# treangenlab/bronko

Measured on AMD Instinct MI355X. Metric: reads/sec through call k-mer->pileup, SARS-CoV-2 k=21, higher is better.
Workload: dtype u64

## Files before the change

### bronko_amd/csrc/bk_engine.cpp

```cpp
#include <hip/hip_runtime.h>

#include <algorithm>
#include <cstdarg>
#include <cstdio>
#include <cstdlib>
#include <cstring>
#include <memory>
#include <string>
#include <vector>

#include "../host/lcb.hpp"
#include "bk_engine.h"

thread_local std::string g_err;

int fail(int code, const char* fmt, ...) {
    char buf[1024];
    va_list ap;
    va_start(ap, fmt);
    vsnprintf(buf, sizeof buf, fmt, ap);
    va_end(ap);
    g_err = buf;
    return code;
}
// ... 32 lines not shown
    BK_HIP(e->n_deferred.alloc(2));
    if (prm->pileup_selected_only && ix.ent_files.p) BK_HIP(e->deferred_mask.alloc(e->deferred.n));
    if (!e->sparse) {
        BK_HIP(e->deferred_n.alloc(e->deferred.n));
        for (MatePlane& p : e->mate) BK_HIP(hipMemset(p.counters.p, 0, std::max<size_t>(p.counters.n, 1) * sizeof(unsigned long long)));
    }
    if (ix.n_files == 1 && !e->sparse && ix.n_full > 0) { BK_HIP(e->lean_e_list.alloc((size_t)ix.n_full)); BK_HIP(e->lean_n_list.alloc(8)); BK_HIP(hipMemset(e->lean_n_list.p, 0, 8 * sizeof(unsigned int))); }
    BK_HIP(e->pileup.alloc(ix.total_cells * 4 * 4));
    e->gather_mode = ix.gather_ok && e->sparse && ix.cell_file.p && ix.dirty_ans.p && ix.W > 1 && ix.file_cell_lo_d.p && !test_env("BK_NO_GATHER");
    if (e->gather_mode) {
        for (MatePlane& p : e->mate) BK_HIP(p.alias_hits.alloc((size_t)bk_engine::kAliasCap * 3));
        BK_HIP(e->n_alias_hits.alloc(2));
        BK_HIP(e->last_sel.upload(std::vector<int>(1, -1)));
        BK_HIP(hipMemset(e->pileup.p, 0, std::max<size_t>(e->pileup.n, 1) * sizeof(unsigned long long)));
        const bool two_pass = prm->pileup_selected_only != 0 && ix.n_files > 1;
        if (!two_pass && prm->cs < (1ull << 28) && ix.total_cells >= 2 * (uint64_t)ix.n_full && !test_env("BK_NO_VOTE_TABLE")) {
            BK_HIP(e->row_bits.alloc((size_t)((bk::v_real_rows(ix.n_full, ix.v_span) + 31) / 32) + 1));
            BK_HIP(e->vote_tab.alloc(bk::vote_table_words(ix.view())));
        }
    }
    BK_HIP(e->stats.alloc((size_t)2 * ix.n_files * 3));
    BK_HIP(e->present.alloc((size_t)2 * ix.n_files));
    if (prm->pileup_selected_only != 0 && ix.n_files > 1) BK_HIP(e->sel_out.alloc(1));
    BK_HIP(e->l2_plan.alloc(4));
    BK_HIP(e->kstats.alloc(8));
    e->use_items = !e->sparse && ix.ref_in_lds && ix.W > 0 && ix.n_lds_bins > 0 && !test_env("BK_NO_ITEMS") && ix.seed_tab2.p && ix.rc_words.p &&
                   bk::item_geometry(std::min<uint32_t>(ix.n_lds_bins, (uint32_t)ix.total_cells), ix.n_full, ix.v_span, &e->ig) &&
                   bk::items_lds_bytes(e->ig, std::min<uint32_t>(ix.n_lds_bins, (uint32_t)ix.total_cells)) <= 128u * 1024u;
    if (e->use_items) {
        if (const char* cp = test_env("BK_ITEM_CAPS")) {
            unsigned ce = 0, cv = 0;
            if (sscanf(cp, "%u,%u", &ce, &cv) == 2 && ce >= 8 && cv >= 8 && ce <= 64 && cv <= 64 && ce % 8 == 0 && cv % 8 == 0) {
                bk::ItemGeom g2 = e->ig;
                g2.cap_e = ce; g2.cap_v = cv; g2.wg_items = g2.n_ebins * ce + g2.n_vbins * cv; g2.wg_stride = g2.wg_items;
                if (bk::items_lds_bytes(g2, std::min<uint32_t>(ix.n_lds_bins, (uint32_t)ix.total_cells)) <= 118u * 1024u) e->ig = g2;
            }
        }
        const size_t g = bk::items_max_grid(ix.n_cus);
        e->ig.grid_max = (uint32_t)g;
        BK_HIP(e->items.alloc(g * e->ig.wg_stride + 64));
        BK_HIP(e->item_tab.alloc(g * ((size_t)e->ig.n_ebins + e->ig.n_vbins)));
        BK_HIP(e->item_gext.alloc(g * ((size_t)e->ig.n_ebins + e->ig.n_vbins) * bk::kItemGCap));
        BK_HIP(e->ov.alloc((size_t)1 << 20));
        BK_HIP(e->ov_n.alloc(4));
        BK_HIP(hipMemset(e->ov_n.p, 0, 4 * sizeof(unsigned long long)));
    } else {
        BK_HIP(e->slabs.alloc((size_t)ix.n_cus * std::max<uint32_t>(ix.n_lds_bins, 1)));
// ... 280 lines not shown
                        m2[0] / n2, m2[1] / n2, m2[2] / n2, m2[3] / n2);
        if (test_env("BK_L2_STATS")[0] == '2')
            for (int b = 0; b < n_wg; b++) fprintf(stderr, "[bk]   wg %d: %.1f %.1f %.1f %.1f\n", b, (clk[4 * b] - t0) * 0.01, (clk[4 * b + 1] - t0) * 0.01, (clk[4 * b + 2] - t0) * 0.01, (clk[4 * b + 3] - t0) * 0.01);
    }
    fprintf(stderr, "[bk] finalize: %u + %u k-mers deferred to the general kernel\n", nd[0], nd[1]);
    if (e->gather_mode) {
        unsigned int ah[2] = {0u, 0u};
        BK_HIP(hipMemcpy(ah, e->n_alias_hits.p, sizeof ah, hipMemcpyDeviceToHost));
        fprintf(stderr, "[bk] votes gathered cell by cell (bk_gather.hip); alias hits among the deferred k-mers: %u + %u\n", ah[0], ah[1]);
    }
    if (e->sparse) {
        unsigned int nl[8];
        BK_HIP(hipMemcpy(nl, e->mate[0].n_list.p, sizeof nl, hipMemcpyDeviceToHost));
        fprintf(stderr, "[bk] sparse finalize (mate file 0): %u V rows of %llu, %u pseudo rows of %llu, %u reference k-mers of %u and %u pseudo k-mers of %u touched\n",
                nl[0], (unsigned long long)bk::v_real_rows(ix.n_full, ix.v_span), nl[4], (unsigned long long)ix.n_prows, nl[2], ix.n_full, nl[3], ix.n_u - ix.n_full);
    }
    fprintf(stderr, "[bk] scan: %llu mismatches counted, %llu items processed, %llu E gaps before a mismatch, %llu behind the last\n", h[23], h[24], h[25], h[26]);
    fprintf(stderr, "[bk] scan N batches: %llu with %llu pieces (%.1f per batch), %llu of them forced by a tile's end\n", h[20], h[21], h[20] ? (double)h[21] / (double)h[20] : 0.0, h[22]);
    fprintf(stderr, "[bk] scan marked: no-diagonal %llu, dirty-head %llu, clean-head %llu, pairs %llu | level 2: k-mers %llu in %llu chunks, simple %llu, dead %llu, "
            "dirty answers %llu (one difference but id unknown: %llu), neither half present %llu, slow %llu (diffs 0/1/2/3+ with a diagonal: %llu/%llu/%llu/%llu) -> member %llu, neighbour %llu, nothing %llu\n",
            h[0], h[1], h[2], h[3], h[4], h[11], h[5], h[6], h[16], h[17], h[18], h[7], h[12], h[13], h[14], h[15], h[8], h[9], h[10]);
    return BK_OK;
}
#else
static int l2_count_report(bk_engine*, const bk::ScanArgs&) { return BK_OK; }
static int l2_stats_arm(bk_engine*) { return BK_OK; }
static int l2_stats_report(bk_engine*) { return BK_OK; }
#endif

static bk::ScanArgs scan_args(const bk_engine* e, int mate, const uint32_t* d_words, uint32_t stride_words, const uint16_t* d_lens, uint64_t n,
                              const unsigned long long* n_records_dev) {
    const IndexTables& ix = *e->ix;
    const MatePlane& pl = e->mate[mate];
    bk::ScanArgs a{};
    a.n_records_dev = n_records_dev; a.ixp = ix.d_view.p;
    a.k = ix.k; a.wstart = ix.wstart; a.W = ix.W; a.v_omin = ix.v_omin; a.v_span = ix.v_span; a.v_off = ix.v_off; a.total_cells = (uint32_t)ix.total_cells; a.n_u = ix.n_u;
    a.ref_words = ix.ref_words.p; a.cell_codes = ix.cell_codes.p; a.cell_has = ix.cell_has.p; a.cell_clean = ix.cell_clean.p; a.cell_clean3 = ix.cell_clean3.p; a.cell_yf = ix.cell_yf.p; a.cell_yr = ix.cell_yr.p; a.id_at = ix.id_at.p; a.cell_fast = ix.cell_fast.p; a.cell_nat = ix.cell_nat.p; a.cell_natrow = ix.cell_natrow.p; a.cell_blk = ix.cell_blk.p; a.seed_tab = ix.seed_tab.p; a.seed_log2 = ix.seed_log2;
    a.seed_tab2 = ix.seed_tab2.p; a.seed2_log2 = ix.seed2_log2; a.rc_words = ix.rc_words.p;
    a.n_direct = e->use_items && ix.n_files == 1 && ix.max_seqs_per_file == 1 && (uint64_t)ix.n_lds_bins >= ix.total_cells && !test_env("BK_NO_N_DIRECT");
    a.words = d_words; a.lens = d_lens; a.n_records = n; a.stride_words = stride_words;
    a.counters = pl.counters.p; a.kmer_total = e->kstats.p + mate * 4 + 1;
    a.ablate = ix.ablate; a.slabs = e->slabs.p; a.n_lds_bins = ix.n_lds_bins; a.ref_in_lds = ix.ref_in_lds ? 1 : 0;
    a.ktab_keys = e->ktab.keys.p; a.ktab_cnt = e->ktab.cnt.p; a.ktab_log2 = e->ktab.log2;
    a.ktab_overflow = e->ktab_out.p + 4; a.mate = (uint32_t)mate;
    a.occ = ix.occ.p; a.n_files = ix.n_files;
    if (e->sparse) {
        a.touch_v = pl.touch_v.p; a.touch_b = pl.touch_b.p; a.touch_p = pl.touch_p.p; a.touch_e = pl.touch_e.p;
        a.rl_recip = ~0ull / (unsigned long long)(ix.v_span + 1) + 1ull;
    }
    a.dbg = e->dbg.p; a.l2_words = bk::scan_l2_words(stride_words, ix.k); a.l2_min_grid = (uint32_t)std::max(1, ix.n_cus / 2);
    if (e->use_items) { a.ig = e->ig; a.items = e->items.p; a.tab = e->item_tab.p; a.gext = e->item_gext.p; a.ov = e->ov.p; a.ov_n = e->ov_n.p; a.ov_cap = (uint32_t)e->ov.n; }
    return a;
}
static int choose_window(bk_engine* e, bk::ScanArgs& a, uint64_t n) {
    const IndexTables& ix = *e->ix;
    if (ix.occ.p && !e->win_chosen && n > 0) {
        BK_HIP(hipMemsetAsync(e->win_votes.p, 0, e->win_votes.n * sizeof(unsigned int), e->stream));
        const char* wf = test_env("BK_WINDOW_FILE");
        const int forced = wf ? std::max(0, atoi(wf)) : -1;
        bk::launch_pick_window(a, 16384, e->win_votes.p, ix.file_cell_lo_d.p, forced, e->win_sel.p, e->stream);
        e->win_chosen = true;
    }
    a.win_dev = ix.occ.p ? e->win_sel.p : nullptr;
    return BK_OK;
}
static uint64_t next_launch(const bk_engine* e, uint64_t left, uint64_t l2_cap, uint32_t& grid) {
    const IndexTables& ix = *e->ix;
    grid = bk::scan_grid(left, ix.n_cus);
    uint64_t take = e->use_items ? std::min<uint64_t>(left, l2_cap) : std::min<uint64_t>(std::min<uint64_t>(left, bk::scan_max_records(grid)), l2_cap);
    if (ix.max_launch_records) take = std::min<uint64_t>(take, ix.max_launch_records);
    if (e->use_items) {
        int share = ix.n_cus - ix.n_cus / 4;
        if (const char* fr = test_env("BK_ITEM_SHARE")) share = std::max(1, std::min(ix.n_cus, ix.n_cus * atoi(fr) / 16));
        grid = bk::items_grid(take, ix.family.load() > 1 ? share : ix.n_cus);
        if (const char* gr = test_env("BK_ITEM_GRID")) grid = std::max<uint32_t>(1, std::min<uint32_t>(grid, (uint32_t)atoi(gr)));
    }
    return take;
}
static int make_l2_room(bk_engine* e, bk::ScanArgs& a, uint64_t l2_cap) {
    if (e->l2_bits.n < a.n_records * a.l2_words || e->l2_diag.n < a.n_records) {
        BK_HIP(hipStreamSynchronize(e->stream));
        const uint64_t recs = std::min<uint64_t>(std::max<uint64_t>(a.n_records + a.n_records / 4, 1 << 16), l2_cap);
        BK_HIP(e->l2_bits.alloc((size_t)recs * a.l2_words)); BK_HIP(e->n_bits.alloc((size_t)recs * a.l2_words)); BK_HIP(e->l2_diag.alloc((size_t)recs));
        BK_HIP(e->l2_any.alloc((size_t)(recs + 31) / 32)); BK_HIP(e->n_any.alloc((size_t)(recs + 31) / 32));
        for (DevBuf<unsigned int>* b : {&e->l2_bits, &e->l2_any, &e->n_bits, &e->n_any}) BK_HIP(hipMemsetAsync(b->p, 0, b->n * sizeof(unsigned int), e->stream));
    }
    a.l2_bits = e->l2_bits.p; a.l2_diag = e->l2_diag.p; a.l2_any = e->l2_any.p; a.n_bits = e->n_bits.p; a.n_any = e->n_any.p;
    return BK_OK;
}
static int bin_items(bk_engine* e, bk::ScanArgs& a, int mate, uint32_t grid, bool wait_v) {
    const IndexTables& ix = *e->ix;
    MatePlane& pl = e->mate[mate];
    bk_engine::Span sp(e, 3);
    bk::BinArgs b{};
    b.ig = e->ig; b.items = e->items.p; b.tab = e->item_tab.p; b.gext = e->item_gext.p; b.n_wg = grid; b.ov = e->ov.p; b.ov_n = e->ov_n.p; b.ov_cap = (uint32_t)e->ov.n;
    b.ov_par = e->ov_par; e->ov_par ^= 1u;
    b.id_at = ix.id_at.p; b.cell_codes = ix.cell_codes.p + bk::scan_ref_pad_words(); b.win_lo = a.win_lo; b.win_dev = a.win_dev; b.total_cells = (uint32_t)ix.total_cells;
    b.counters = pl.counters.p; b.v_off = ix.v_off; b.v_real_len = bk::v_real_len(ix.n_full, ix.v_span); b.rl = (uint32_t)ix.v_span + 1u;
    const bool v_clean = pl.take_v_clean();
    b.v_mode = ix.item_v_mode >= 0 ? ix.item_v_mode : (v_clean ? 2 : 1);
    if (const char* ba = test_env("BK_BIN_ABLATE")) b.ablate = atoi(ba);
    if (wait_v) {
        e->pending.on = true; e->pending.mate = mate; e->pending.b = b;
        b.part = 1;
        a.touch_v = pl.fuse_touch.p; a.rl_recip = ~0ull / (unsigned long long)(ix.v_span + 1) + 1ull;
        pl.items_wait();
    } else {
        pl.no_more_waiting();
        if (e->fuse_ok) a.touch_v = nullptr;
    }
    BK_HIP(bk::launch_bin_count(b, e->stream));
    return BK_OK;
}
static int level2_and_fold(bk_engine* e, const bk::ScanArgs& a, int mate, uint32_t grid) {
    const IndexTables& ix = *e->ix;
    bk_engine::Span sp(e, 3);
    if (int rc = l2_count_report(e, a)) return rc;
    if (ix.ablate == 1 || ix.ablate == 4) {
        BK_HIP(hipMemsetAsync(e->n_bits.p, 0, (size_t)a.n_records * a.l2_words * sizeof(unsigned int), e->stream));
        BK_HIP(hipMemsetAsync(e->n_any.p, 0, e->n_any.n * sizeof(unsigned int), e->stream));
    }
    else BK_HIP(bk::launch_level2(a, ix.n_cus, e->stream));
    if (!e->use_items) {
        bk::FoldArgs f{};
        f.slabs = e->slabs.p; f.n_slabs = grid; f.n_lds_bins = ix.n_lds_bins; f.id_at = ix.id_at.p; f.cell_codes = ix.cell_codes.p + bk::scan_ref_pad_words(); f.win_lo = a.win_lo; f.win_dev = a.win_dev; f.touch_e = a.touch_e;
        f.counters = e->mate[mate].counters.p;
        bk::launch_fold(f, e->stream);
    }
    return BK_OK;
}
static int push_device(bk_engine* e, int mate, const uint32_t* d_words, uint32_t stride_words, const uint16_t* d_lens, uint64_t n,
                       const unsigned long long* n_records_dev = nullptr, uint64_t kmers_upper = 0) {
    MatePlane& pl = e->mate[mate];
    if (int rc = pl.zero_if_stale(e)) return rc;
    const uint64_t upper = kmers_upper ? kmers_upper : n * (uint64_t)stride_words * 16;
    if (int rc = ensure_ktab_room(e, upper)) return rc;
    if (e->dump) { if (int rc = dump_push(e, mate, d_words, stride_words, d_lens, n, n_records_dev, upper)) return rc; }
    pl.written();
    if (int rc = l2_stats_arm(e)) return rc;
    bk::ScanArgs a = scan_args(e, mate, d_words, stride_words, d_lens, n, n_records_dev);
    if (e->ix->W <= 0) {
        bk::launch_count_kmers(a, e->stream);
    } else {
        if (int rc = choose_window(e, a, n)) return rc;
        const uint64_t l2_cap = std::max<uint64_t>(64, ((1ull << 30) / sizeof(unsigned int)) / a.l2_words);
        for (uint64_t base = 0; base < n; base += a.n_records) {
            uint32_t grid = 0;
            a.rec_base = base; a.n_records = next_launch(e, n - base, l2_cap, grid);
            if (int rc = make_l2_room(e, a, l2_cap)) return rc;
            if (int rc = flush_pending_items(e)) return rc;
            const bool wait_v = e->fuse_ok && a.n_direct && !pl.fuse_off && e->ix->item_v_mode < 0;
            a.l2_plan = e->use_items && e->ix->n_files == 1 && e->ix->family.load() >= 4 && !test_env("BK_NO_L2_PLAN") ? e->l2_plan.p : nullptr;
            {
                bk_engine::Span sp(e, 0);
                if (e->use_items) { a.ov_par = e->ov_par; BK_HIP(bk::launch_scan_items(a, grid, e->stream)); }
                else BK_HIP(bk::launch_scan_count(a, grid, e->stream));
            }
            if (e->use_items) { if (int rc = bin_items(e, a, mate, grid, wait_v)) return rc; }
            if (int rc = level2_and_fold(e, a, mate, grid)) return rc;
        }
    }
    BK_HIP(hipGetLastError());
    if (!n_records_dev) pl.pushed_records += n;
    return note_ktab_fill(e);
}

static constexpr int kPush = 1;
static int push_checks(bk_engine* e, int mate, uint64_t n, bool batch_ok, const char* bad_batch, bool too_large) {
    if (!e) return fail(BK_ERR_INVALID, "null engine");
    if (!e->in_sample) return fail(BK_ERR_STATE, "bk_push_reads_* called before bk_sample_begin");
    if (mate < 0 || mate > 1) return fail(BK_ERR_INVALID, "mate must be 0 or 1");
    if (n == 0) return BK_OK;
    if (!batch_ok) return fail(BK_ERR_INVALID, "%s", bad_batch);
    if (too_large) return fail(BK_ERR_INVALID, "batch too large: push at most 2^32 bases per call");
    BK_HIP(hipSetDevice(e->device));
    return kPush;
}
static int packed_checks(bk_engine* e, int mate, const void* words, uint32_t stride_words, const void* lens, uint64_t n) {
    return push_checks(e, mate, n, words && lens && stride_words != 0 && stride_words <= 4096, "bad record batch",
                       stride_words != 0 && n > (1ull << 32) / ((uint64_t)stride_words * 16));
}
struct PackGeom {
// ... 781 lines not shown
```

### bronko_amd/csrc/bk_engine.h

```cpp
#pragma once
#include <hip/hip_runtime.h>

#include <algorithm>
#include <atomic>
#include <chrono>
#include <cstdio>
#include <cstdlib>
#include <memory>
#include <string>
#include <thread>
#include <vector>

#include "../../include/bronko_hip.h"
#include "bk_device.h"
#include "bk_kernels.h"

#pragma GCC visibility push(hidden)

extern thread_local std::string g_err;

int fail(int code, const char* fmt, ...);

#define BK_HIP(expr)                                                                                  \
    do {                                                                                              \
// ... 210 lines not shown
    DevBuf<unsigned int> xchg_cnt;
    bool ktab_exchanged = false;
    std::unique_ptr<KmerDump> dump;
    bool gather_mode = false;
    DevBuf<unsigned int> row_bits;
    DevBuf<uint32_t> vote_tab;
    DevBuf<unsigned int> n_alias_hits;
    static constexpr unsigned int kAliasCap = 1u << 20;
    DevBuf<int> last_sel;
    DevBuf<unsigned int> slabs;
    bool use_items = false;
    bk::ItemGeom ig{};
    DevBuf<unsigned short> items, item_tab;
    DevBuf<unsigned short> item_gext;
    DevBuf<unsigned int> ov;
    DevBuf<unsigned long long> ov_n;
    uint32_t ov_par = 0;
    DevBuf<unsigned int> lean_e_list, lean_n_list;
    bool fuse_ok = false;
    struct PendingItems { bool on = false; int mate = 0; bk::BinArgs b{}; } pending;
    DevBuf<unsigned int> n_bits, n_any;
    DevBuf<unsigned int> l2_bits;
    DevBuf<unsigned int> l2_any;
    DevBuf<unsigned int> l2_plan;
    DevBuf<uint2> l2_diag;
    bool sparse = false;
    DevBuf<unsigned long long> pileup;
    DevBuf<unsigned long long> stats;
    DevBuf<unsigned char> present;
    DevBuf<unsigned long long> kstats;
    struct StageSlot {
        DevBuf<uint32_t> words; DevBuf<uint16_t> lens;
        uint8_t* h = nullptr; size_t h_cap = 0;
        hipEvent_t done = nullptr; bool busy = false;
    } stage[2];
    int next_stage = 0;

    struct IngestSlot {
        uint8_t* h_bases = nullptr; size_t h_bases_cap = 0;
        unsigned long long* h_off = nullptr; size_t h_off_cap = 0;
        DevBuf<uint8_t> d_bases;
        uint8_t* h_quals = nullptr; size_t h_quals_cap = 0;
        DevBuf<uint8_t> d_quals;
        DevBuf<unsigned long long> d_off, d_nrec;
        DevBuf<uint32_t> d_work;
        DevBuf<uint32_t> d_words;
        DevBuf<uint16_t> d_lens;
// ... 45 lines not shown
```

### bronko_amd/csrc/bk_kernels.h

```cpp
#pragma once
#include <hip/hip_runtime.h>

#include "../../include/bronko_hip.h"
#include "bk_device.h"

namespace bk {

struct ItemGeom {
    uint32_t n_ebins, n_vbins;
    uint32_t cap_e, cap_v;
    uint32_t vq_log2;
    uint32_t wg_items;
    uint32_t wg_stride;
    uint32_t grid_max;
};
constexpr uint32_t kEBinLog2 = 7;
constexpr uint32_t kERunMax = 255;
constexpr uint32_t kEBinSpan = (1u << kEBinLog2) + kERunMax;
constexpr uint32_t kItemGCap = 256;

struct ScanArgs {
    const IndexView* ixp;
    int32_t k, wstart, W, v_omin, v_span;
    uint64_t v_off;
// ... 7 lines not shown
    const uint32_t* cell_yr;
    const uint32_t* id_at;
    const uint32_t* cell_fast;
    const uint2* cell_blk;
    const uint32_t* cell_nat;
    const uint32_t* cell_natrow;
    const uint2* seed_tab;
    uint32_t seed_log2;
    const uint2* seed_tab2;
    uint32_t seed2_log2;
    const uint32_t* rc_words;
    const uint32_t* words;
    const uint16_t* lens;
    uint64_t rec_base;
    uint64_t n_records;
    const unsigned long long* n_records_dev;
    uint32_t stride_words;
    unsigned long long* counters;
    unsigned int* slabs;
    unsigned int* n_bits;
    unsigned int* n_any;
    unsigned int* l2_bits;
    unsigned int* l2_any;
    unsigned int* l2_plan;
    uint32_t l2_min_grid;
    uint2* l2_diag;
    uint32_t l2_words;
    uint32_t n_lds_bins;
    uint32_t win_lo;
    const uint32_t* win_dev;
    const uint32_t* occ;
    int32_t win_file, n_files;
    int ref_in_lds;
    unsigned long long* kmer_total;
    unsigned long long* ktab_keys;
    unsigned int* ktab_cnt;
    uint32_t ktab_log2;
    unsigned long long* ktab_overflow;
    uint32_t mate;
    unsigned int* touch_v;
    unsigned int* touch_b;
    unsigned int* touch_p;
    unsigned int* touch_e;
    unsigned long long rl_recip;
    ItemGeom ig;
    unsigned short* items;
    unsigned short* tab;
// ... 114 lines not shown
hipError_t launch_level2(const ScanArgs& a, int n_cus, hipStream_t stream);
hipError_t launch_scan_count(const ScanArgs& a, uint32_t grid, hipStream_t stream);
void launch_fold(const FoldArgs& f, hipStream_t stream);
struct BinArgs {
    ItemGeom ig;
    const unsigned short* items;
    const unsigned short* tab;
    const unsigned short* gext;
    uint32_t n_wg;
    const unsigned int* ov;
    unsigned long long* ov_n;
    uint32_t ov_cap, ov_par;
    const uint32_t* id_at;
    const uint32_t* cell_codes;
    uint32_t win_lo;
    const uint32_t* win_dev;
    uint32_t total_cells;
    unsigned long long* counters;
    uint64_t v_off, v_real_len;
    uint32_t rl;
    int v_mode;
    int part;
    int ablate;
};
bool item_geometry(uint32_t win_cells, uint32_t n_full, int v_span, ItemGeom* g);
uint32_t items_grid(uint64_t n_records, int n_cus);
uint32_t items_max_grid(int n_cus);
size_t items_lds_bytes(const ItemGeom& g, uint32_t win_cells);
hipError_t launch_scan_items(const ScanArgs& a, uint32_t grid, hipStream_t stream);
hipError_t launch_bin_count(const BinArgs& b, hipStream_t stream);
void launch_ktab_stats(const unsigned long long* keys, const unsigned int* cnt, uint32_t log2n, unsigned long long ci,
                       unsigned long long cx, unsigned long long* out, hipStream_t stream);
void launch_ktab_rehash(const unsigned long long* okeys, const unsigned int* ocnt, uint32_t olog2, unsigned long long* nkeys, unsigned int* ncnt,
                        uint32_t nlog2, unsigned long long* overflow, hipStream_t stream);
void launch_ktab_count_parts(const unsigned long long* keys, uint32_t log2n, uint32_t n_parts, unsigned long long* counts, hipStream_t stream);
void launch_ktab_scatter_parts(const unsigned long long* keys, const unsigned int* cnt, uint32_t log2n, uint32_t n_parts, unsigned long long* cursors,
                               unsigned long long* out_keys, unsigned int* out_cnt, hipStream_t stream);
void launch_ktab_import(const unsigned long long* in_keys, const unsigned int* in_cnt, uint64_t n, unsigned long long* keys, unsigned int* cnt, uint32_t log2n,
                        unsigned long long* overflow, hipStream_t stream);
void launch_ktab_totals_to_kstats(unsigned long long* ktab_out, unsigned long long* kstats, int n_mates, hipStream_t stream);
uint32_t ktab_fill_words();
void launch_kmer_dump_count(const uint32_t* words, const uint16_t* lens, uint64_t n_records, const unsigned long long* n_records_dev,
                            uint32_t stride_words, int k, uint32_t mate, unsigned long long* keys, unsigned int* cnt, uint32_t log2n,
                            unsigned long long* overflow, int n_cus, hipStream_t stream);
void launch_kmer_dump_select(const unsigned long long* keys, const unsigned int* cnt, uint32_t log2n, uint32_t mate, unsigned long long ci,
                             unsigned long long cs, unsigned long long cx, unsigned long long* out_keys, unsigned int* out_cnt, uint64_t cap,
// ... 74 lines not shown
```

### bronko_amd/csrc/bk_kernels.hip

```cpp
#include <hip/hip_runtime.h>

#include <algorithm>
#include <cstdlib>
#include <mutex>
#include <utility>
#include <vector>

#include "bk_device.h"
#include "bk_kernels.h"
#include "bk_scan_common.h"
#include "bk_finalize_common.h"

namespace bk {


__device__ __forceinline__ int probe_table(const TableSlot* __restrict__ sub, uint32_t log2s, uint64_t key) {
    const uint32_t smask = (1u << log2s) - 1u;
    uint32_t h = hash_key(key, log2s);
    for (;;) {
        const uint4 e = *reinterpret_cast<const uint4*>(sub + h);
        const uint64_t kk = (uint64_t)e.x | ((uint64_t)e.y << 32);
        if (kk == key) return (int)e.z;
        if (kk == kEmptyKey) return -1;
        h = (h + 1) & smask;
// ... 1504 lines not shown
                    const uint32_t base = qk + incl - p;
                    if (fits) {
                        uint32_t x = bits, i = 0;
                        while (x) {
                            const uint32_t bpos = (uint32_t)__builtin_ctz(x);
                            x &= x - 1u;
                            kq[base + i++] = ((unsigned long long)rec << 16) | ((w0 + (uint32_t)j) * 32u + bpos);
                        }
                        bits = 0u;
                    }
                    const unsigned long long fm = __ballot(fits);
                    const uint32_t taken = fm ? (uint32_t)__shfl((int)incl, 63 - __builtin_clzll(fm)) : 0u;
                    qk += taken;
                    __builtin_amdgcn_wave_barrier();
                    while (qk >= 64u) take_kmers();
                }
            }
        }
    };

    const uint64_t n_any = (n_records + 31) / 32;
    const uint64_t n_blk = (n_any + kAnyWords - 1) / kAnyWords;

    const uint32_t g_work = a.l2_plan ? min((uint32_t)gridDim.x, max(*a.l2_plan, 1u)) : (uint32_t)gridDim.x;
    if (blockIdx.x >= g_work) return;
    for (uint64_t blk = (uint64_t)blockIdx.x * kL2Waves + wave; blk < n_blk; blk += (uint64_t)g_work * kL2Waves) {
        const uint64_t i = blk * kAnyWords + lane;
        const uint32_t anyw = (lane < kAnyWords && i < n_any) ? a.l2_any[i] : 0u;
        if (anyw) a.l2_any[i] = 0u;
        if (!__ballot(anyw != 0u)) continue;
#pragma unroll
        for (int j = 0; j < kAnyWords / 2; ++j) {
            const uint32_t wv = (uint32_t)__shfl((int)anyw, 2 * j + (lane >> 5));
            const bool marked = (wv >> (lane & 31)) & 1u;
            const unsigned long long hm = __ballot(marked);
            if (hm) {
                if (marked) rq[qr + lane_prefix(hm)] = (uint32_t)(blk * (kAnyWords * 32) + 64u * (uint32_t)j + (uint32_t)lane);
                qr += (uint32_t)__popcll(hm);
                __builtin_amdgcn_wave_barrier();
                if (qr >= 64u) take_records();
            }
        }
    }
    while (qr) take_records();
    while (qk) take_kmers();
    while (qn) slow_batch();
}

__global__ __launch_bounds__(256) void pick_window_kernel(ScanArgs a, uint64_t n_probe, unsigned int* votes) {
// ... 93 lines not shown
#define BK_PICK(KT) (!a.touch_v ? (a.ref_in_lds ? scan_count_kernel<true, KT, false> : scan_count_kernel<false, KT, false>) \
                                : (a.ref_in_lds ? scan_count_kernel<true, KT, true> : scan_count_kernel<false, KT, true>))
    kern = a.k == 21 ? BK_PICK(21) : a.k == 31 ? BK_PICK(31) : BK_PICK(0);
#undef BK_PICK
    {
        static std::mutex mu;
        static std::vector<std::pair<std::pair<const void*, int>, size_t>> have;
        int dev = 0;
        (void)hipGetDevice(&dev);
        const void* fn = reinterpret_cast<const void*>(kern);
        std::lock_guard<std::mutex> lock(mu);
        size_t* cur = nullptr;
        for (auto& h : have) if (h.first.first == fn && h.first.second == dev) cur = &h.second;
        if (!cur || *cur < lds) {
            hipError_t e = hipFuncSetAttribute(fn, hipFuncAttributeMaxDynamicSharedMemorySize, (int)lds);
            if (e != hipSuccess) return e;
            if (cur) *cur = lds; else have.push_back({{fn, dev}, lds});
        }
    }
    hipLaunchKernelGGL(kern, dim3(grid), dim3(kScanBlock), lds, stream, a);
    return hipGetLastError();
}

__global__ __launch_bounds__(1024) void l2_plan_kernel(const unsigned int* __restrict__ l2_any, uint64_t n_words, unsigned int* __restrict__ plan, uint32_t g_min) {
    __shared__ unsigned int part[16];
    unsigned int n = 0;
    for (uint64_t i = threadIdx.x; i < n_words; i += 1024u) n += (unsigned int)__popc(l2_any[i]);
#pragma unroll
    for (int off = 32; off; off >>= 1) n += (unsigned int)__shfl_xor((int)n, off);
    if ((threadIdx.x & 63u) == 0u) part[threadIdx.x >> 6] = n;
    __syncthreads();
    if (threadIdx.x == 0) {
        unsigned int t = 0;
        for (int w = 0; w < 16; ++w) t += part[w];
        plan[0] = max(g_min, (t + 255u) / 256u);
    }
}

hipError_t launch_level2(const ScanArgs& a, int n_cus, hipStream_t stream) {
    if (a.n_records == 0 || a.W <= 0) return hipSuccess;
    const bool stats = a.ktab_keys != nullptr;
    void (*kern)(ScanArgs);
    if (!a.n_direct) {
#define BK_PICKN(KT) (!a.touch_v ? (stats ? nbatch_kernel<true, KT, false> : nbatch_kernel<false, KT, false>) \
                                 : (stats ? nbatch_kernel<true, KT, true> : nbatch_kernel<false, KT, true>))
        kern = a.k == 21 ? BK_PICKN(21) : a.k == 31 ? BK_PICKN(31) : BK_PICKN(0);
#undef BK_PICKN
        const uint64_t turns = (a.n_records + 32 * kAnyWords * kNbBlocksPerWave - 1) / (32 * kAnyWords * kNbBlocksPerWave);
        const unsigned grid = (unsigned)std::max<uint64_t>(1, std::min<uint64_t>((turns + kL2Waves - 1) / kL2Waves, (uint64_t)n_cus * 8));
        hipLaunchKernelGGL(kern, dim3(grid), dim3(kL2Block), 0, stream, a);
    }
#define BK_PICK(KT) (!a.touch_v ? (stats ? level2_kernel<true, KT, false> : level2_kernel<false, KT, false>) \
                                : (stats ? level2_kernel<true, KT, true> : level2_kernel<false, KT, true>))
    kern = a.k == 21 ? BK_PICK(21) : a.k == 31 ? BK_PICK(31) : BK_PICK(0);
#undef BK_PICK
    const uint64_t blks = (a.n_records + 32 * kAnyWords - 1) / (32 * kAnyWords);
    const unsigned grid = (unsigned)std::max<uint64_t>(1, std::min<uint64_t>((blks + kL2Waves - 1) / kL2Waves, (uint64_t)n_cus * (a.n_files == 1 ? 2 : 8)));
    if (a.l2_plan) hipLaunchKernelGGL(l2_plan_kernel, dim3(1), dim3(1024), 0, stream, (const unsigned int*)a.l2_any, (a.n_records + 31) / 32, a.l2_plan, a.l2_min_grid);
    hipLaunchKernelGGL(kern, dim3(grid), dim3(kL2Block), 0, stream, a);
    return hipGetLastError();
}

__global__ __launch_bounds__(256) void fold_kernel(FoldArgs f) {
    const uint64_t tid = (uint64_t)blockIdx.x * 256 + threadIdx.x;
    const uint64_t nthreads = (uint64_t)gridDim.x * 256;
    const uint32_t per = (f.n_slabs + gridDim.y - 1) / gridDim.y;
    const uint32_t b0 = blockIdx.y * per, b1 = min(f.n_slabs, b0 + per);
    for (uint64_t i = tid; i < f.n_lds_bins && b0 < b1; i += nthreads) {
        unsigned long long s0 = 0, s1 = 0;
        for (uint32_t b = b0; b < b1; ++b) {
            const unsigned int v = f.slabs[(size_t)b * f.n_lds_bins + i];
            s0 += v & 0xffffu;
            s1 += v >> 16;
        }
        if (s0 | s1) {
            const uint64_t cell = (f.win_dev ? f.win_dev[1] : f.win_lo) + i;
            const uint32_t id = f.id_at[cell];
            const uint32_t rc = ((f.cell_codes[cell >> 4] >> (2 * (cell & 15))) & 3u) == 2u ? 1u : 0u;
            touch(f.touch_e, id);
            if (s0) atomicAdd(f.counters + 2 * (size_t)id + rc, s0);
            if (s1) atomicAdd(f.counters + 2 * (size_t)id + (1u - rc), s1);
// ... 1166 lines not shown
```

### bronko_amd/csrc/bk_scan_items.hip

```cpp
#include <hip/hip_runtime.h>

#include <algorithm>
#include <mutex>
#include <utility>
#include <vector>

#include "bk_device.h"
#include "bk_kernels.h"
#include "bk_scan_common.h"

namespace bk {

constexpr int kItemBlock = 1024;
constexpr int kItemWaves = kItemBlock / 64;
constexpr int kItemGroupsPerCu = 1;
constexpr uint32_t kListCap = 256;
constexpr uint32_t kListWords = kListCap + 4u;
constexpr uint32_t kDealRing = 32;
constexpr size_t kItemLdsFixed = (4 + 4 + 2 * kDealRing + kItemWaves * kListWords) * sizeof(unsigned int);
constexpr int kBinBlock = 256;
constexpr uint32_t kMaxChunkMismatches = 24;
constexpr uint32_t kStageMaxWords = 12;

__device__ __forceinline__ void item_direct(const __attribute__((address_space(4))) ScanArgs* ap, uint32_t bin, uint32_t item, uint32_t win_lo) {
// ... 575 lines not shown
    }
    BK_DBG_CLOCK2(a, 3);
    uint32_t tot = nkm;
#pragma unroll
    for (int off = 32; off; off >>= 1) tot += (uint32_t)__shfl_xor((int)tot, off);
    if (lane == 0 && tot) atomicAdd(block_kmers, tot);
    __syncthreads();
    if (threadIdx.x == 0 && *block_kmers) { unsigned long long* kt = cold()->kmer_total; if (kt) atomicAdd(kt, (unsigned long long)*block_kmers); }
    BK_DBG_CLOCK(a, 3);
}

__global__ __launch_bounds__(kBinBlock) void bin_count_kernel(BinArgs b) {
    extern __shared__ __attribute__((aligned(16))) unsigned int acc[];
    const uint32_t n_eb = b.ig.n_ebins, n_bins = n_eb + b.ig.n_vbins, bin = blockIdx.x + (b.part == 2 ? n_eb : 0u);
    const bool is_e = bin < n_eb;
    const uint32_t vsize = (6u << b.ig.vq_log2) * b.rl;
    const uint32_t n_acc = is_e ? 2u * (kEBinSpan + 1u) : vsize;
    const int lane = threadIdx.x & 63;
    const int wave = __builtin_amdgcn_readfirstlane((int)(threadIdx.x >> 6));
    if (BK_ABLATE(b, 5)) return;
    const uint32_t cap = is_e ? b.ig.cap_e : b.ig.cap_v;
    const uint32_t G = b.ig.grid_max;
    const unsigned short* const bin_items = b.items + (is_e ? (size_t)bin * G * b.ig.cap_e : (size_t)n_eb * G * b.ig.cap_e + (size_t)(bin - n_eb) * G * b.ig.cap_v);
    const bool mine = threadIdx.x < b.n_wg && !BK_ABLATE(b, 1);
    const unsigned short* reg0 = bin_items + (size_t)(mine ? threadIdx.x : 0u) * cap;
    uint32_t hdr0 = 0u;
    uint4 v0 = make_uint4(0u, 0u, 0u, 0u), v1 = v0, v2 = v0, v3 = v0, v4 = v0, v5 = v0;
    if (mine) {
        const uint4* q = reinterpret_cast<const uint4*>(reg0);
        hdr0 = b.tab[(size_t)bin * G + threadIdx.x];
        v0 = q[0]; v1 = q[1]; v2 = q[2];
        if (is_e) { v3 = q[3]; v4 = q[4]; v5 = q[5]; }
    }
    for (uint32_t i = threadIdx.x; i < n_acc; i += kBinBlock) acc[i] = 0u;
    if (BK_ABLATE(b, 6)) return;
    if (bin == 0 && threadIdx.x == 0) b.ov_n[b.ov_par ^ 1u] = 0ull;
    __syncthreads();
    auto take = [&](uint32_t it) __attribute__((always_inline)) {
        if (it == 0xffffu) return;
        if (is_e) {
            const uint32_t c = it & 127u, n = ((it >> 7) & 255u) + 1u;
            unsigned int* d = acc + (it >> 15) * (kEBinSpan + 1u);
            __hip_atomic_fetch_add(d + c, 1u, __ATOMIC_RELAXED, __HIP_MEMORY_SCOPE_WORKGROUP);
            __hip_atomic_fetch_add(d + c + n, 0u - 1u, __ATOMIC_RELAXED, __HIP_MEMORY_SCOPE_WORKGROUP);
        } else {
            __hip_atomic_fetch_add(acc + (it & 0x7fffu), (it & 0x8000u) ? 0u - 1u : 1u, __ATOMIC_RELAXED, __HIP_MEMORY_SCOPE_WORKGROUP);
        }
    };
    auto take8 = [&](const uint4& v, uint32_t left) __attribute__((always_inline)) {
        if (left > 0u) take(v.x & 0xffffu);
        if (left > 1u) take(v.x >> 16);
        if (left > 2u) take(v.y & 0xffffu);
        if (left > 3u) take(v.y >> 16);
        if (left > 4u) take(v.z & 0xffffu);
        if (left > 5u) take(v.z >> 16);
        if (left > 6u) take(v.w & 0xffffu);
        if (left > 7u) take(v.w >> 16);
    };
    auto take_items = [&](const unsigned short* p, uint32_t n) __attribute__((always_inline)) {
        const uint4* q = reinterpret_cast<const uint4*>(p);
// ... 29 lines not shown
        const uint32_t n_all = b.tab[(size_t)bin * G + wg], n = min(n_all, cap);
        take_items(bin_items + (size_t)wg * cap, n);
        take_items(b.gext + ((size_t)wg * n_bins + bin) * kItemGCap, min(n_all - n, kItemGCap));
    }
    if (g_mine) {
        const uint4* q = reinterpret_cast<const uint4*>(b.gext + ((size_t)threadIdx.x * n_bins + bin) * kItemGCap);
        const uint4 z = make_uint4(0u, 0u, 0u, 0u);
        for (uint32_t i0 = 0; i0 < g_mine; i0 += 128u) {
            uint4 u[16];
#pragma unroll
            for (uint32_t j = 0; j < 16u; ++j) u[j] = i0 + 8u * j < g_mine ? q[(i0 >> 3) + j] : z;
#pragma unroll
            for (uint32_t j = 0; j < 16u; ++j) take8(u[j], g_mine > i0 + 8u * j ? g_mine - i0 - 8u * j : 0u);
        }
    }
    if (!BK_ABLATE(b, 7)) {
        const unsigned long long n_all = b.ov_n[b.ov_par];
        const uint32_t n_ov = (uint32_t)(n_all < (unsigned long long)b.ov_cap ? n_all : (unsigned long long)b.ov_cap);
        for (uint32_t i = threadIdx.x; i < n_ov; i += kBinBlock) {
            const uint32_t e = b.ov[i];
            if ((e >> 16) == bin) take(e & 0xffffu);
        }
    }
    __syncthreads();
    if (is_e) {
        if (wave < 2) {
            unsigned int* d = acc + (uint32_t)wave * (kEBinSpan + 1u) + (uint32_t)lane * 6u;
            const uint32_t d0 = d[0], d1 = d[1], d2 = d[2], d3 = d[3], d4 = d[4], d5 = d[5];
            const uint32_t sum = d0 + d1 + d2 + d3 + d4 + d5;
            uint32_t inc = sum;
#pragma unroll
            for (int off = 1; off < 64; off <<= 1) { const uint32_t t = (uint32_t)__shfl_up((int)inc, off); if (lane >= off) inc += t; }
            uint32_t run = inc - sum;
            run += d0; d[0] = run; run += d1; d[1] = run; run += d2; d[2] = run; run += d3; d[3] = run; run += d4; d[4] = run; run += d5; d[5] = run;
        }
        __syncthreads();
        const uint32_t win_lo = b.win_dev ? b.win_dev[1] : b.win_lo;
        for (uint32_t i = threadIdx.x; i < kEBinSpan && !BK_ABLATE(b, 2) && !BK_ABLATE(b, 3); i += kBinBlock) {
            const uint32_t s0 = acc[i], s1 = acc[(kEBinSpan + 1u) + i];
            if (s0 | s1) {
                const uint32_t cell = win_lo + (bin << kEBinLog2) + i;
                const uint32_t id = b.id_at[cell];
                const uint32_t rc = ((b.cell_codes[cell >> 4] >> (2u * (cell & 15u))) & 3u) == 2u ? 1u : 0u;
                if (s0) atomicAdd(b.counters + 2 * (size_t)id + rc, (unsigned long long)s0);
                if (s1) atomicAdd(b.counters + 2 * (size_t)id + (1u - rc), (unsigned long long)s1);
            }
        }
// ... 99 lines not shown
```

Measured before the change: 8.662 billion.

## Build compact list of marked records in bin kernel to drive level-2 work

Replaces the separate single-block l2_plan kernel (popcount of l2_any to size the level-2 grid) with a compaction step inside the bin-count kernel. That step turns the l2_any bitmap into a dense list of marked record indices using per-block popcount, prefix sums and an atomic offset. Level 2 then walks the list directly, with per-wave shares sized by a records-per-wave knob, instead of sweeping the whole bitmap. This removes a serial one-block launch and the bitmap sweep, at the cost of extra global atomics and scattered writes in the bin kernel, plus a counter reset done by the last block.

```diff
diff --git a/bronko_amd/csrc/bk_engine.cpp b/bronko_amd/csrc/bk_engine.cpp
--- a/bronko_amd/csrc/bk_engine.cpp
+++ b/bronko_amd/csrc/bk_engine.cpp
@@ -78,7 +78,6 @@
     BK_HIP(e->stats.alloc((size_t)2 * ix.n_files * 3));
     BK_HIP(e->present.alloc((size_t)2 * ix.n_files));
     if (prm->pileup_selected_only != 0 && ix.n_files > 1) BK_HIP(e->sel_out.alloc(1));
-    BK_HIP(e->l2_plan.alloc(4));
     BK_HIP(e->kstats.alloc(8));
     e->use_items = !e->sparse && ix.ref_in_lds && ix.W > 0 && ix.n_lds_bins > 0 && !test_env("BK_NO_ITEMS") && ix.seed_tab2.p && ix.rc_words.p &&
                    bk::item_geometry(std::min<uint32_t>(ix.n_lds_bins, (uint32_t)ix.total_cells), ix.n_full, ix.v_span, &e->ig) &&
@@ -405,7 +404,31 @@
             h[0], h[1], h[2], h[3], h[4], h[11], h[5], h[6], h[16], h[17], h[18], h[7], h[12], h[13], h[14], h[15], h[8], h[9], h[10]);
     return BK_OK;
 }
+static int l2_check_clean(bk_engine* e, const bk::ScanArgs& a) {
+    if (!test_env("BK_L2_CHECK_CLEAN")) return BK_OK;
+    BK_HIP(hipStreamSynchronize(e->stream));
+    std::vector<unsigned int> h;
+    const struct { const char* what; const unsigned int* p; size_t n; } bufs[] = {
+        {"l2_any", e->l2_any.p, e->l2_any.n}, {"l2_bits", e->l2_bits.p, (size_t)a.n_records * a.l2_words}, {"the list's count", e->l2_list_n.p, e->l2_list_n.n}};
+    for (const auto& b : bufs) {
+        h.assign(b.n, 0u);
+        if (b.n) BK_HIP(hipMemcpy(h.data(), b.p, b.n * sizeof(unsigned int), hipMemcpyDeviceToHost));
+        for (size_t i = 0; i < b.n; ++i) if (h[i]) return fail(BK_ERR_STATE, "Level 2 left %s not zero (word %zu = %u)", b.what, i, h[i]);
+    }
+    return BK_OK;
+}
+static int l2_list_expect(bk_engine* e, const bk::ScanArgs& a) {
+    const char* want = test_env("BK_L2_LIST_EXPECT");
+    if (!want) return BK_OK;
+    BK_HIP(hipStreamSynchronize(e->stream));
+    unsigned int n = 0;
+    BK_HIP(hipMemcpy(&n, e->l2_list_n.p, sizeof n, hipMemcpyDeviceToHost));
+    if ((n != 0u) != (atoi(want) != 0)) return fail(BK_ERR_STATE, "the scan listed %u marked records (list %s)", n, a.l2_list ? "on" : "off");
+    return BK_OK;
+}
 #else
+static int l2_list_expect(bk_engine*, const bk::ScanArgs&) { return BK_OK; }
+static int l2_check_clean(bk_engine*, const bk::ScanArgs&) { return BK_OK; }
 static int l2_count_report(bk_engine*, const bk::ScanArgs&) { return BK_OK; }
 static int l2_stats_arm(bk_engine*) { return BK_OK; }
 static int l2_stats_report(bk_engine*) { return BK_OK; }
@@ -431,7 +454,10 @@
         a.touch_v = pl.touch_v.p; a.touch_b = pl.touch_b.p; a.touch_p = pl.touch_p.p; a.touch_e = pl.touch_e.p;
         a.rl_recip = ~0ull / (unsigned long long)(ix.v_span + 1) + 1ull;
     }
-    a.dbg = e->dbg.p; a.l2_words = bk::scan_l2_words(stride_words, ix.k); a.l2_min_grid = (uint32_t)std::max(1, ix.n_cus / 2);
+    a.dbg = e->dbg.p; a.l2_words = bk::scan_l2_words(stride_words, ix.k);
+    a.l2_min_grid = (uint32_t)std::max(1, ix.n_cus / 2); a.l2_rec_per_wave = ix.family.load() >= 4 ? 64 : 8;
+    if (const char* v = test_env("BK_L2_MIN_GRID")) a.l2_min_grid = (uint32_t)std::max(1, atoi(v));
+    if (const char* v = test_env("BK_L2_REC_PER_WAVE")) a.l2_rec_per_wave = (uint32_t)std::max(1, atoi(v));
     if (e->use_items) { a.ig = e->ig; a.items = e->items.p; a.tab = e->item_tab.p; a.gext = e->item_gext.p; a.ov = e->ov.p; a.ov_n = e->ov_n.p; a.ov_cap = (uint32_t)e->ov.n; }
     return a;
 }
@@ -466,9 +492,13 @@
         const uint64_t recs = std::min<uint64_t>(std::max<uint64_t>(a.n_records + a.n_records / 4, 1 << 16), l2_cap);
         BK_HIP(e->l2_bits.alloc((size_t)recs * a.l2_words)); BK_HIP(e->n_bits.alloc((size_t)recs * a.l2_words)); BK_HIP(e->l2_diag.alloc((size_t)recs));
         BK_HIP(e->l2_any.alloc((size_t)(recs + 31) / 32)); BK_HIP(e->n_any.alloc((size_t)(recs + 31) / 32));
-        for (DevBuf<unsigned int>* b : {&e->l2_bits, &e->l2_any, &e->n_bits, &e->n_any}) BK_HIP(hipMemsetAsync(b->p, 0, b->n * sizeof(unsigned int), e->stream));
+        BK_HIP(e->l2_list.alloc((size_t)recs)); BK_HIP(e->l2_list_n.alloc(2));
+        for (DevBuf<unsigned int>* b : {&e->l2_bits, &e->l2_any, &e->n_bits, &e->n_any, &e->l2_list_n}) BK_HIP(hipMemsetAsync(b->p, 0, b->n * sizeof(unsigned int), e->stream));
     }
     a.l2_bits = e->l2_bits.p; a.l2_diag = e->l2_diag.p; a.l2_any = e->l2_any.p; a.n_bits = e->n_bits.p; a.n_any = e->n_any.p;
+    const bool sweep = test_env("BK_L2_SWEEP") || test_env("BK_NO_L2_PLAN") || e->ix->ablate == 1 || e->ix->ablate == 4;
+    const bool listed = e->use_items && a.n_direct && e->ix->n_files == 1 && !e->ktab.keys.p && !sweep;
+    a.l2_list = listed ? e->l2_list.p : nullptr; a.l2_list_n = e->l2_list_n.p; a.l2_list_cap = listed ? (uint32_t)std::min<size_t>(e->l2_list.n, 0xffffffffu) : 0u;
     return BK_OK;
 }
 static int bin_items(bk_engine* e, bk::ScanArgs& a, int mate, uint32_t grid, bool wait_v) {
@@ -492,6 +522,7 @@
         pl.no_more_waiting();
         if (e->fuse_ok) a.touch_v = nullptr;
     }
+    if (a.l2_list) { b.l2_any = a.l2_any; b.l2_words = (uint32_t)((a.n_records + 31) / 32); b.l2_list = a.l2_list; b.l2_list_n = a.l2_list_n; b.l2_list_cap = a.l2_list_cap; }
     BK_HIP(bk::launch_bin_count(b, e->stream));
     return BK_OK;
 }
@@ -533,14 +564,15 @@
             if (int rc = make_l2_room(e, a, l2_cap)) return rc;
             if (int rc = flush_pending_items(e)) return rc;
             const bool wait_v = e->fuse_ok && a.n_direct && !pl.fuse_off && e->ix->item_v_mode < 0;
-            a.l2_plan = e->use_items && e->ix->n_files == 1 && e->ix->family.load() >= 4 && !test_env("BK_NO_L2_PLAN") ? e->l2_plan.p : nullptr;
             {
                 bk_engine::Span sp(e, 0);
                 if (e->use_items) { a.ov_par = e->ov_par; BK_HIP(bk::launch_scan_items(a, grid, e->stream)); }
                 else BK_HIP(bk::launch_scan_count(a, grid, e->stream));
             }
             if (e->use_items) { if (int rc = bin_items(e, a, mate, grid, wait_v)) return rc; }
+            if (int rc = l2_list_expect(e, a)) return rc;
             if (int rc = level2_and_fold(e, a, mate, grid)) return rc;
+            if (int rc = l2_check_clean(e, a)) return rc;
         }
     }
     BK_HIP(hipGetLastError());
diff --git a/bronko_amd/csrc/bk_engine.h b/bronko_amd/csrc/bk_engine.h
--- a/bronko_amd/csrc/bk_engine.h
+++ b/bronko_amd/csrc/bk_engine.h
@@ -256,7 +256,7 @@
     DevBuf<unsigned int> n_bits, n_any;
     DevBuf<unsigned int> l2_bits;
     DevBuf<unsigned int> l2_any;
-    DevBuf<unsigned int> l2_plan;
+    DevBuf<unsigned int> l2_list, l2_list_n;
     DevBuf<uint2> l2_diag;
     bool sparse = false;
     DevBuf<unsigned long long> pileup;
diff --git a/bronko_amd/csrc/bk_kernels.h b/bronko_amd/csrc/bk_kernels.h
--- a/bronko_amd/csrc/bk_kernels.h
+++ b/bronko_amd/csrc/bk_kernels.h
@@ -53,7 +53,10 @@
     unsigned int* n_any;
     unsigned int* l2_bits;
     unsigned int* l2_any;
-    unsigned int* l2_plan;
+    unsigned int* l2_list;
+    unsigned int* l2_list_n;
+    uint32_t l2_list_cap;
+    uint32_t l2_rec_per_wave;
     uint32_t l2_min_grid;
     uint2* l2_diag;
     uint32_t l2_words;
@@ -214,6 +217,11 @@
     int v_mode;
     int part;
     int ablate;
+    const unsigned int* l2_any;
+    uint32_t l2_words;
+    unsigned int* l2_list;
+    unsigned int* l2_list_n;
+    uint32_t l2_list_cap;
 };
 bool item_geometry(uint32_t win_cells, uint32_t n_full, int v_span, ItemGeom* g);
 uint32_t items_grid(uint64_t n_records, int n_cus);
diff --git a/bronko_amd/csrc/bk_kernels.hip b/bronko_amd/csrc/bk_kernels.hip
--- a/bronko_amd/csrc/bk_kernels.hip
+++ b/bronko_amd/csrc/bk_kernels.hip
@@ -1550,9 +1550,32 @@
     const uint64_t n_any = (n_records + 31) / 32;
     const uint64_t n_blk = (n_any + kAnyWords - 1) / kAnyWords;
 
-    const uint32_t g_work = a.l2_plan ? min((uint32_t)gridDim.x, max(*a.l2_plan, 1u)) : (uint32_t)gridDim.x;
-    if (blockIdx.x >= g_work) return;
-    for (uint64_t blk = (uint64_t)blockIdx.x * kL2Waves + wave; blk < n_blk; blk += (uint64_t)g_work * kL2Waves) {
+    if (a.l2_list) {
+        const uint32_t n_list = min(*a.l2_list_n, a.l2_list_cap);
+        if (n_list == 0u) return;
+        const uint32_t per_wg = max(a.l2_rec_per_wave, 1u) * kL2Waves;
+        const uint32_t g_work = min((uint32_t)gridDim.x, max((n_list + per_wg - 1u) / per_wg, max(a.l2_min_grid, 1u)));
+        if (blockIdx.x >= g_work) return;
+        const uint32_t share = (n_list + g_work * kL2Waves - 1u) / (g_work * kL2Waves);
+        const uint32_t i0 = min((blockIdx.x * kL2Waves + (uint32_t)wave) * share, n_list), i1 = min(i0 + share, n_list);
+        for (uint32_t i = i0; i < i1; i += 64u) {
+            const uint32_t m = min(i1 - i, 64u);
+            if ((uint32_t)lane < m) {
+                const uint32_t rec = a.l2_list[i + (uint32_t)lane];
+                atomicAnd(a.l2_any + (rec >> 5), ~(1u << (rec & 31u)));
+                rq[lane] = rec;
+            }
+            qr = m;
+            __builtin_amdgcn_wave_barrier();
+            take_records();
+        }
+        while (qk) take_kmers();
+        while (qn) slow_batch();
+        __syncthreads();
+        if (threadIdx.x == 0 && atomicInc(a.l2_list_n + 1, g_work - 1u) == g_work - 1u) a.l2_list_n[0] = 0u;
+        return;
+    }
+    for (uint64_t blk = (uint64_t)blockIdx.x * kL2Waves + wave; blk < n_blk; blk += (uint64_t)gridDim.x * kL2Waves) {
         const uint64_t i = blk * kAnyWords + lane;
         const uint32_t anyw = (lane < kAnyWords && i < n_any) ? a.l2_any[i] : 0u;
         if (anyw) a.l2_any[i] = 0u;
@@ -1692,21 +1715,6 @@
     return hipGetLastError();
 }
 
-__global__ __launch_bounds__(1024) void l2_plan_kernel(const unsigned int* __restrict__ l2_any, uint64_t n_words, unsigned int* __restrict__ plan, uint32_t g_min) {
-    __shared__ unsigned int part[16];
-    unsigned int n = 0;
-    for (uint64_t i = threadIdx.x; i < n_words; i += 1024u) n += (unsigned int)__popc(l2_any[i]);
-#pragma unroll
-    for (int off = 32; off; off >>= 1) n += (unsigned int)__shfl_xor((int)n, off);
-    if ((threadIdx.x & 63u) == 0u) part[threadIdx.x >> 6] = n;
-    __syncthreads();
-    if (threadIdx.x == 0) {
-        unsigned int t = 0;
-        for (int w = 0; w < 16; ++w) t += part[w];
-        plan[0] = max(g_min, (t + 255u) / 256u);
-    }
-}
-
 hipError_t launch_level2(const ScanArgs& a, int n_cus, hipStream_t stream) {
     if (a.n_records == 0 || a.W <= 0) return hipSuccess;
     const bool stats = a.ktab_keys != nullptr;
@@ -1726,7 +1734,6 @@
 #undef BK_PICK
     const uint64_t blks = (a.n_records + 32 * kAnyWords - 1) / (32 * kAnyWords);
     const unsigned grid = (unsigned)std::max<uint64_t>(1, std::min<uint64_t>((blks + kL2Waves - 1) / kL2Waves, (uint64_t)n_cus * (a.n_files == 1 ? 2 : 8)));
-    if (a.l2_plan) hipLaunchKernelGGL(l2_plan_kernel, dim3(1), dim3(1024), 0, stream, (const unsigned int*)a.l2_any, (a.n_records + 31) / 32, a.l2_plan, a.l2_min_grid);
     hipLaunchKernelGGL(kern, dim3(grid), dim3(kL2Block), 0, stream, a);
     return hipGetLastError();
 }
diff --git a/bronko_amd/csrc/bk_scan_items.hip b/bronko_amd/csrc/bk_scan_items.hip
--- a/bronko_amd/csrc/bk_scan_items.hip
+++ b/bronko_amd/csrc/bk_scan_items.hip
@@ -621,6 +621,17 @@
     const uint32_t cap = is_e ? b.ig.cap_e : b.ig.cap_v;
     const uint32_t G = b.ig.grid_max;
     const unsigned short* const bin_items = b.items + (is_e ? (size_t)bin * G * b.ig.cap_e : (size_t)n_eb * G * b.ig.cap_e + (size_t)(bin - n_eb) * G * b.ig.cap_v);
+    __shared__ unsigned int l2s[kBinBlock / 64 + 1];
+    const uint32_t l2_per = b.l2_list ? (b.l2_words + gridDim.x - 1u) / gridDim.x : 0u;
+    const uint32_t l2_w0 = min(blockIdx.x * l2_per, b.l2_words), l2_w1 = min(l2_w0 + l2_per, b.l2_words);
+    uint32_t l2_mine = 0u, l2_incl = 0u;
+    if (l2_w0 < l2_w1) {
+        for (uint32_t w = l2_w0 + threadIdx.x; w < l2_w1; w += kBinBlock) l2_mine += (uint32_t)__popc(b.l2_any[w]);
+        l2_incl = l2_mine;
+#pragma unroll
+        for (int off = 1; off < 64; off <<= 1) { const uint32_t t = (uint32_t)__shfl_up((int)l2_incl, off); if (lane >= off) l2_incl += t; }
+        if (lane == 63) l2s[wave] = l2_incl;
+    }
     const bool mine = threadIdx.x < b.n_wg && !BK_ABLATE(b, 1);
     const unsigned short* reg0 = bin_items + (size_t)(mine ? threadIdx.x : 0u) * cap;
     uint32_t hdr0 = 0u;
@@ -635,6 +646,12 @@
     if (BK_ABLATE(b, 6)) return;
     if (bin == 0 && threadIdx.x == 0) b.ov_n[b.ov_par ^ 1u] = 0ull;
     __syncthreads();
+    uint32_t l2_at = 0u;
+    if (l2_w0 < l2_w1 && threadIdx.x == 0) {
+        uint32_t t = 0u;
+        for (int w = 0; w < kBinBlock / 64; ++w) t += l2s[w];
+        if (t) l2_at = atomicAdd(b.l2_list_n, t);
+    }
     auto take = [&](uint32_t it) __attribute__((always_inline)) {
         if (it == 0xffffu) return;
         if (is_e) {
@@ -710,7 +727,21 @@
             if ((e >> 16) == bin) take(e & 0xffffu);
         }
     }
+    if (l2_w0 < l2_w1 && threadIdx.x == 0) l2s[kBinBlock / 64] = l2_at;
     __syncthreads();
+    if (l2_w0 < l2_w1 && l2_mine) {
+        uint32_t at = l2s[kBinBlock / 64] + l2_incl - l2_mine;
+        for (int w = 0; w < wave; ++w) at += l2s[w];
+        for (uint32_t w = l2_w0 + threadIdx.x; w < l2_w1; w += kBinBlock) {
+            uint32_t bits = b.l2_any[w];
+            while (bits) {
+                const uint32_t bp = (uint32_t)__builtin_ctz(bits);
+                bits &= bits - 1u;
+                if (at < b.l2_list_cap) b.l2_list[at] = w * 32u + bp;
+                ++at;
+            }
+        }
+    }
     if (is_e) {
         if (wave < 2) {
             unsigned int* d = acc + (uint32_t)wave * (kEBinSpan + 1u) + (uint32_t)lane * 6u;
```

Result: faster. 9.168 billion (median of 6 runs) (+5.8%).
